# applied-ai-lab/genesis

Hardware: AMD Instinct MI355X
Metric: training images/sec (fwd+bwd+GECO step), GENESIS-V2 K=7 64x64 (higher is better)
Workload: dtype f32

## Files before the change

genesis_amd/csrc/gx_norm.hip:

```cpp
#include "gx_common.h"

#include <vector>

namespace {

struct View {
    float* ptr;
    int ctot;
    int c0;
    int mode;
    const float* proj;
    int projC;
    const float* pgate;
    int nsplit;
    size_t sstride;
};

struct InSrc {
    const float* p;
    int nsplit;
    size_t stride;
    const float* bias;
    float* ysum;
};
// ... 759 lines not shown
    double s1 = 0.0, s2 = 0.0;
    for (int tc = 0; tc < cpg; ++tc) {
        double a = 0.0, b = 0.0;
        for (int p = 0; p < P; ++p) { a += uab[2 * (tc * P + p)]; b += uab[2 * (tc * P + p) + 1]; }
        const float gmc = gamma[gidx * cpg + tc];
        s1 += b * gmc;
        s2 += a * gmc;
        if ((int)threadIdx.x == tc) {
            float* pp = part_out + ((size_t)n * C + gidx * cpg + tc) * 3;
            pp[0] = (float)a; pp[1] = (float)b;
        }
    }
    const float k1 = (float)(s1 / m), k2 = (float)(s2 / m);
    float sd = 0.f, am = 0.f;
    float gm2 = gm, bt2 = bt;
    asm volatile("" : "+v"(gm2), "+v"(bt2));
    float wacc[CT];
#pragma unroll
    for (int q = 0; q < CT; ++q) wacc[q] = 0.f;
#pragma unroll
    for (int j = 0; j < F; ++j) {
        int jo = j * 64;
        static_assert(CT == 4, "the dependency list below names four accumulators");
        if (WP) asm volatile("" : "+v"(jo) : "v"(sd), "v"(am), "v"(k1), "v"(wacc[0]), "v"(wacc[1]), "v"(wacc[2]), "v"(wacc[3]));
        else asm volatile("" : "+v"(jo) : "v"(sd), "v"(am), "v"(k1));
        f32x4 g = {0.f, 0.f, 0.f, 0.f}, o, a;
        f32x4& xv = xr[KEEP ? j : 0];
        if constexpr (!KEEP) {
            xv = src4[jo];
#pragma unroll
            for (int e = 0; e < 4; ++e) xv[e] = (xv[e] - meanf) * rstdf;
        }
#pragma unroll
        for (int e = 0; e < 4; ++e) {
            const float t = xv[e] * gm2 + bt2;
            a[e] = t > 0.f ? t : 0.f;
        }
#pragma unroll
        for (int q = 0; q < CT; ++q) {
            const f32x4 gq = gs4[q * rowq + jo];
            g += pw[q] * gq;
            if (WP) wacc[q] += (gq[0] * a[0] + gq[1] * a[1]) + (gq[2] * a[2] + gq[3] * a[3]);
        }
#pragma unroll
        for (int e = 0; e < 4; ++e) {
            const float pre = xv[e] * gm2 + bt2;
            const float gv = pre > 0.f ? g[e] : 0.f;
            const float d = rstdf * (gv * gm2 - k1 - xv[e] * k2);
            o[e] = d;
        }
        sd += (o[0] + o[1]) + (o[2] + o[3]);
        am = fmaxf(fmaxf(am, fmaxf(fabsf(o[0]), fabsf(o[1]))), fmaxf(fabsf(o[2]), fabsf(o[3])));
        dst4[jo] = o;
    }
    {
        const double v = gx_wave_sum_d((double)sd);
        if (lane == 0) usd[unit] = v;
#pragma unroll
        for (int of = 32; of >= 1; of >>= 1) am = fmaxf(am, __shfl_xor(am, of, 64));
        if (lane == 0) uam[unit] = am;
    }
    if (WP) {
#pragma unroll
        for (int q = 0; q < CT; ++q) {
            float v = wacc[q];
#pragma unroll
            for (int o = 32; o >= 1; o >>= 1) v += __shfl_xor(v, o, 64);
            if (lane == 0) uw[unit][q] = v;
        }
    }
    __syncthreads();
    if (WP) {
        for (int t = threadIdx.x; t < cpg * ctot; t += blockDim.x) {
            const int tc = t / ctot, q = t - tc * ctot;
            float v = 0.f;
            for (int p = 0; p < P; ++p) v += uw[tc * P + p][q];
            wpart[((size_t)n * ctot + q) * C + gidx * cpg + tc] = v;
        }
    }
    if ((int)threadIdx.x < cpg) {
        double s = 0.0;
        for (int p = 0; p < P; ++p) s += usd[threadIdx.x * P + p];
        part_out[((size_t)n * C + gidx * cpg + threadIdx.x) * 3 + 2] = (float)s;
    }
    if (amax_parts && threadIdx.x == 0) {
        float r = uam[0];
#pragma unroll
        for (int i = 1; i < 16; ++i) r = fmaxf(r, uam[i]);
        amax_parts[blockIdx.x] = r;
    }
}

__global__ void __launch_bounds__(1024)
gn_relu_fwd_small_kernel(const InSrc src, const float* __restrict__ gamma, const float* __restrict__ beta,
                         int C, int H, int W, int groups, float eps, View d0, View d1,
                         float* __restrict__ mean_out, float* __restrict__ rstd_out) {
    __shared__ double red[16 * 2 + 2];
    const int n = blockIdx.x / groups, gidx = blockIdx.x % groups;
    const int cpg = C / groups, HW = H * W;
    const int m = cpg * HW;
    const int e = threadIdx.x * 4;
    const bool act = e < m;
    const size_t slab_off = ((size_t)n * C + (size_t)gidx * cpg) * HW;
    f32x4 v = {0.f, 0.f, 0.f, 0.f};
    if (act) v = load_in4(src, slab_off + e, gidx * cpg + e / HW);
    double acc[2];
    acc[0] = ((double)v[0] + (double)v[1]) + ((double)v[2] + (double)v[3]);
    acc[1] = ((double)v[0] * v[0] + (double)v[1] * v[1]) + ((double)v[2] * v[2] + (double)v[3] * v[3]);
    block_sum_multi<2>(acc, red);
    const double mean = acc[0] / m;
    double var = acc[1] / m - mean * mean;
    if (var < 0.0) var = 0.0;
    const float meanf = (float)mean;
    const float rstdf = (float)(1.0 / sqrt(var + (double)eps));
    if (threadIdx.x == 0) { mean_out[blockIdx.x] = meanf; rstd_out[blockIdx.x] = rstdf; }
    if (act && d0.ptr) {
        const int cl = e / HW, hw = e - cl * HW;
        const int c = gidx * cpg + cl;
        const int r = hw / W, col = hw - r * W;
        const float gm = gamma[c], bt = beta[c];
        f32x4 o;
#pragma unroll
        for (int u = 0; u < 4; ++u) {
            const float t = (v[u] - meanf) * rstdf * gm + bt;
            o[u] = t > 0.f ? t : 0.f;
        }
        store_view4(d0, n, c, r, col, H, W, o);
        if (d1.ptr) store_view4(d1, n, c, r, col, H, W, o);
    }
}

__global__ void __launch_bounds__(1024)
gn_relu_bwd_small_kernel(const float* __restrict__ y, const float* __restrict__ gamma, const float* __restrict__ beta,
                         const float* __restrict__ mean_in, const float* __restrict__ rstd_in,
                         int C, int H, int W, int groups, View g0, View g1,
                         float* __restrict__ dy, float* __restrict__ part_out) {
    __shared__ double ta[1024], tb[1024];
    __shared__ double ca[64], cb[64];
    const int n = blockIdx.x / groups, gidx = blockIdx.x % groups;
    const int cpg = C / groups, HW = H * W;
    const int m = cpg * HW;
    const int tpc = HW >> 2;
    const int e = threadIdx.x * 4;
    const bool act = e < m;
    const size_t slab_off = ((size_t)n * C + (size_t)gidx * cpg) * HW;
    const float meanf = mean_in[blockIdx.x], rstdf = rstd_in[blockIdx.x];
    int cl = 0, c = gidx * cpg, r = 0, col = 0;
    f32x4 xh = {0.f, 0.f, 0.f, 0.f}, gv = {0.f, 0.f, 0.f, 0.f};
    float gm = 0.f;
    double a = 0.0, b = 0.0;
    if (act) {
        cl = e / HW;
        const int hw = e - cl * HW;
        c = gidx * cpg + cl;
        r = hw / W; col = hw - r * W;
        const f32x4 xv = reinterpret_cast<const f32x4*>(y + slab_off)[threadIdx.x];
        f32x4 g = load_view4(g0, n, c, r, col, H, W);
        if (g1.ptr) { const f32x4 g2 = load_view4(g1, n, c, r, col, H, W); g += g2; }
        gm = gamma[c];
        const float bt = beta[c];
#pragma unroll
        for (int u = 0; u < 4; ++u) {
            const float h = (xv[u] - meanf) * rstdf;
            const float pre = h * gm + bt;
            const float gg = pre > 0.f ? g[u] : 0.f;
            xh[u] = h; gv[u] = gg;
            a += (double)gg * h;
            b += (double)gg;
        }
    }
    ta[threadIdx.x] = a; tb[threadIdx.x] = b;
    __syncthreads();
    if ((int)threadIdx.x < cpg) {
        double sa = 0.0, sb = 0.0;
        for (int i = 0; i < tpc; ++i) { sa += ta[threadIdx.x * tpc + i]; sb += tb[threadIdx.x * tpc + i]; }
        ca[threadIdx.x] = sa; cb[threadIdx.x] = sb;
        float* pp = part_out + ((size_t)n * C + gidx * cpg + threadIdx.x) * 3;
        pp[0] = (float)sa; pp[1] = (float)sb;
    }
    __syncthreads();
    double s1 = 0.0, s2 = 0.0;
    for (int i = 0; i < cpg; ++i) {
        const float gi = gamma[gidx * cpg + i];
        s1 += cb[i] * gi;
        s2 += ca[i] * gi;
    }
    const float k1 = (float)(s1 / m), k2 = (float)(s2 / m);
    double sd = 0.0;
    if (act) {
        f32x4 o;
#pragma unroll
        for (int u = 0; u < 4; ++u) {
            const float d = rstdf * (gv[u] * gm - k1 - xh[u] * k2);
            o[u] = d;
            sd += d;
        }
        reinterpret_cast<f32x4*>(dy + slab_off)[threadIdx.x] = o;
    }
    __syncthreads();
    ta[threadIdx.x] = sd;
    __syncthreads();
    if ((int)threadIdx.x < cpg) {
        double s = 0.0;
        for (int i = 0; i < tpc; ++i) s += ta[threadIdx.x * tpc + i];
        part_out[((size_t)n * C + gidx * cpg + threadIdx.x) * 3 + 2] = (float)s;
    }
}

int small_threads(int cpg, int H, int W) {
    const int HW = H * W, m = cpg * HW;
    if (HW >= 256 || (W % 4) != 0 || cpg > 64 || m > 4096) return 0;
    return gx_round_up(m / 4, 64);
}

inline float* gn_take_link_out(const float* tensor, int ctot, int c0, int mode, int C, unsigned nwg, size_t covered, bool second_copy = false) {
    GxAmaxLink& L = gx_amax_link();
    const bool link_ok = !second_copy && L.parts && !L.tensor && tensor && c0 == 0 && mode == 0 && ctot == C && covered == L.numel;
    return gx_amax_producer_out(tensor, link_ok, nwg, covered);
}
template <int F, int UPW>
void launch_fwd_reg(dim3 grid, dim3 block, hipStream_t s, const InSrc src, const float* gamma, const float* beta, int C, int H,
                    int W, int groups, int P, float eps, View d0, View d1, float* mean, float* rstd) {
    float* ap = d0.ptr ? gn_take_link_out(d0.ptr, d0.ctot, d0.c0, d0.mode, C, grid.x, (size_t)(grid.x / groups) * C * H * W, d1.ptr != nullptr) : nullptr;
    hipLaunchKernelGGL((gn_relu_fwd_reg_kernel<F, UPW>), grid, block, 0, s, src, gamma, beta, C, H, W, groups, P, eps, d0, d1,
                       mean, rstd, ap);
}
template <int F, int UPW>
bool launch_bwd_stage(dim3 grid, dim3 block, hipStream_t s, size_t lds, const float* y, const float* gamma,
                      const float* beta, const float* mean, const float* rstd, int C, int H, int W, int groups, int P,
                      View g0, View g1, float* dy, float* part, float* wpart, float* bpart) {
    if (UPW != 1 || block.x != 1024 || g0.ctot != 4) return false;
    float* amax_parts = gn_take_link_out(dy, C, 0, 0, C, grid.x, (size_t)(grid.x / groups) * C * H * W);
    constexpr bool KEEP = F < 8;
    static bool attr_set = false;
    if (!attr_set) {
        (void)hipFuncSetAttribute(reinterpret_cast<const void*>(&gn_relu_bwd_stage_kernel<F, 4, true, KEEP>),
                                  hipFuncAttributeMaxDynamicSharedMemorySize, 150 * 1024);
        (void)hipFuncSetAttribute(reinterpret_cast<const void*>(&gn_relu_bwd_stage_kernel<F, 4, false, KEEP>),
                                  hipFuncAttributeMaxDynamicSharedMemorySize, 150 * 1024);
        attr_set = true;
    }
#define GX_STAGE_LAUNCH(WP_)                                                                                               \
    hipLaunchKernelGGL((gn_relu_bwd_stage_kernel<F, 4, WP_, KEEP>), grid, block, lds, s, y, gamma, beta, mean, rstd, C, H, W, \
                       groups, P, g0, g1, dy, part, wpart, bpart, amax_parts)
    if (wpart) GX_STAGE_LAUNCH(true); else GX_STAGE_LAUNCH(false);
#undef GX_STAGE_LAUNCH
    return true;
}

template <int F, int UPW>
void launch_bwd_reg(dim3 grid, dim3 block, hipStream_t s, size_t lds, const float* y, const float* gamma, const float* beta,
                    const float* mean, const float* rstd, int C, int H, int W, int groups, int P, View g0, View g1, float* dy,
                    float* part, float* wpart, float* bpart) {
    if (!lds) {
        float* ap = gn_take_link_out(dy, C, 0, 0, C, grid.x, (size_t)(grid.x / groups) * C * H * W);
        hipLaunchKernelGGL((gn_relu_bwd_reg_kernel<F, UPW, false>), grid, block, 0, s, y, gamma, beta, mean, rstd, C, H, W, groups,
                           P, g0, g1, dy, part, wpart, bpart, ap);
        return;
    }
    static bool attr_set = false;
    if (!attr_set) {
        (void)hipFuncSetAttribute(reinterpret_cast<const void*>(&gn_relu_bwd_reg_kernel<F, UPW, true>),
                                  hipFuncAttributeMaxDynamicSharedMemorySize, 150 * 1024);
        attr_set = true;
    }
    if (launch_bwd_stage<F, UPW>(grid, block, s, lds, y, gamma, beta, mean, rstd, C, H, W, groups, P, g0, g1, dy, part, wpart, bpart))
        return;
    float* ap = gn_take_link_out(dy, C, 0, 0, C, grid.x, (size_t)(grid.x / groups) * C * H * W);
    hipLaunchKernelGGL((gn_relu_bwd_reg_kernel<F, UPW, true>), grid, block, lds, s, y, gamma, beta, mean, rstd, C, H, W, groups, P,
                       g0, g1, dy, part, wpart, bpart, ap);
}

#define GX_GN_REG_DISPATCH(LAUNCH, pl, ...)                                      \
    do {                                                                         \
        if (pl.UPW == 1) {                                                       \
            if (pl.F == 1) LAUNCH<1, 1>(__VA_ARGS__);                            \
            else if (pl.F == 2) LAUNCH<2, 1>(__VA_ARGS__);                       \
            else if (pl.F == 4) LAUNCH<4, 1>(__VA_ARGS__);                       \
            else LAUNCH<8, 1>(__VA_ARGS__);                                      \
        } else {                                                                 \
            if (pl.F == 1) LAUNCH<1, 2>(__VA_ARGS__);                            \
            else if (pl.F == 2) LAUNCH<2, 2>(__VA_ARGS__);                       \
            else LAUNCH<4, 2>(__VA_ARGS__);                                      \
        }                                                                        \
    } while (0)

struct GnRedTable { GxGnRed e[48]; };
__global__ void __launch_bounds__(256)
gn_param_reduce_batch_kernel(const GnRedTable tab) {
    const GxGnRed& r = tab.e[blockIdx.y];
    const int c = blockIdx.x;
    if (c >= r.C) return;
    __shared__ double red[16 * 3 + 3];
    double v[3] = {0.0, 0.0, 0.0};
    for (int n = threadIdx.x; n < r.N; n += blockDim.x) {
        const float* p = r.part + ((size_t)n * r.C + c) * 3;
        v[0] += p[0]; v[1] += p[1]; v[2] += p[2];
    }
    block_sum_multi<3>(v, red);
    if (threadIdx.x == 0) {
        r.dgamma[c] += (float)v[0];
        r.dbeta[c] += (float)v[1];
        if (r.dbias) r.dbias[c] += (float)v[2];
    }
}

int check_view(const char* name, const View& v, int C) {
    GX_CHECK_ARG(v.mode >= 0 && v.mode <= 2, "%s: bad view mode %d", name, v.mode);
    GX_CHECK_ARG(v.c0 >= 0 && v.c0 + C <= v.ctot, "%s: view slice [%d,%d) outside %d channels", name, v.c0,
                 v.c0 + C, v.ctot);
    return GX_OK;
}

constexpr int kSplitPix = 4096;
constexpr int kSplitRec = 3 * 8 + 8 * 8 + 8;
// ... 282 lines not shown
         d1{dst1, dst1_ctot, dst1_c0, dst1_mode, nullptr, 0, nullptr};
    int rc = dst0 ? check_view("gx_gn_relu_fwd", d0, C) : GX_OK;
    if (rc) return rc;
    if (dst1) { rc = check_view("gx_gn_relu_fwd", d1, C); if (rc) return rc; }
    const int m = (C / groups) * H * W;
    const int threads = m >= 16384 ? 1024 : (m >= 2048 ? 512 : 256);
    const bool vec = (W % 4) == 0;
    {
        auto vw = [](int mode) { return mode == 1 ? 4.0 : (mode == 2 ? 0.25 : 1.0); };
        const double el = (double)N * C * H * W;
        GxProf pf(KID_GN_FWD, (hipStream_t)stream, 8.0 * el,
                  4.0 * el * (src.nsplit + (src.ysum ? 1.0 : 0.0) + (dst0 ? vw(dst0_mode) : 0.0) +
                              (dst1 ? vw(dst1_mode) : 0.0)));
        const RegPlan pl = plan_reg(C / groups, H, W);
        const int st = small_threads(C / groups, H, W);
        if (pl.ok)
            GX_GN_REG_DISPATCH(launch_fwd_reg, pl, dim3(N * groups), dim3(pl.threads), (hipStream_t)stream, src, gamma,
                               beta, C, H, W, groups, pl.P, eps, d0, d1, mean, rstd);
        else if (st)
            hipLaunchKernelGGL(gn_relu_fwd_small_kernel, dim3(N * groups), dim3(st), 0, (hipStream_t)stream, src, gamma,
                               beta, C, H, W, groups, eps, d0, d1, mean, rstd);
        else {
            float* ap = dst0 ? gn_take_link_out(dst0, d0.ctot, d0.c0, d0.mode, C, (unsigned)(N * groups), (size_t)N * C * H * W, dst1 != nullptr) : nullptr;
            if (vec)
                hipLaunchKernelGGL(gn_relu_fwd_kernel<true>, dim3(N * groups), dim3(threads), 0, (hipStream_t)stream, src,
                                   gamma, beta, C, H, W, groups, eps, d0, d1, mean, rstd, ap);
            else
                hipLaunchKernelGGL(gn_relu_fwd_kernel<false>, dim3(N * groups), dim3(threads), 0, (hipStream_t)stream, src,
                                   gamma, beta, C, H, W, groups, eps, d0, d1, mean, rstd, ap);
        }
    }
    GX_CHECK_LAUNCH("gx_gn_relu_fwd");
    return GX_OK;
}

size_t gx_gn_relu_bwd_ws_bytes(int N, int C) { return (size_t)N * C * 3 * sizeof(float); }
size_t gx_gn_relu_bwd_proj_ws_bytes(int N, int C, int H, int W, int groups, int Cout) {
    size_t b = gx_gn_relu_bwd_ws_bytes(N, C);
    if (proj_split_ok(C, H, W, groups, Cout))
        b += ((size_t)N * groups * (H * W / kSplitPix) * kSplitRec + (size_t)N * groups * 2) * sizeof(float);
    return b;
}

static int gn_relu_bwd_impl(const float* y, const float* gamma, const float* beta, const float* mean,
                            const float* rstd, int N, int C, int H, int W, int groups, const View& v0, const View& v1,
                            float* dy, float* dgamma, float* dbeta, float* dbias, void* ws, size_t ws_bytes,
                            gx_stream_t stream, float* wpart = nullptr, float* bpart = nullptr);

int gx_gn_relu_bwd(const float* y, const float* gamma, const float* beta, const float* mean, const float* rstd,
                   int N, int C, int H, int W, int groups, const float* g0, int g0_ctot, int g0_c0, int g0_mode,
                   const float* g1, int g1_ctot, int g1_c0, int g1_mode, float* dy, float* dgamma, float* dbeta,
                   float* dbias, void* ws, size_t ws_bytes, gx_stream_t stream) {
    return gx_gn_relu_bwd_parts(y, gamma, beta, mean, rstd, N, C, H, W, groups, g0, g0_ctot, g0_c0, g0_mode, 1, 0, g1, g1_ctot,
                                g1_c0, g1_mode, 1, 0, dy, dgamma, dbeta, dbias, ws, ws_bytes, stream);
}

int gx_gn_relu_bwd_parts(const float* y, const float* gamma, const float* beta, const float* mean, const float* rstd,
                         int N, int C, int H, int W, int groups, const float* g0, int g0_ctot, int g0_c0, int g0_mode,
                         int g0_nsplit, size_t g0_split_stride, const float* g1, int g1_ctot, int g1_c0, int g1_mode,
                         int g1_nsplit, size_t g1_split_stride, float* dy, float* dgamma, float* dbeta, float* dbias, void* ws,
                         size_t ws_bytes, gx_stream_t stream) {
    GX_CHECK_ARG(g0, "gx_gn_relu_bwd: null pointer");
    GX_CHECK_ARG(g0_nsplit >= 1 && g1_nsplit >= 1, "gx_gn_relu_bwd_parts: nsplit >= 1");
    View v0{const_cast<float*>(g0), g0_ctot, g0_c0, g0_mode, nullptr, 0, nullptr, g0_nsplit, g0_split_stride},
         v1{const_cast<float*>(g1), g1_ctot, g1_c0, g1_mode, nullptr, 0, nullptr, g1_nsplit, g1_split_stride};
    int rc = check_view("gx_gn_relu_bwd", v0, C);
    if (rc) return rc;
    if (g1) { rc = check_view("gx_gn_relu_bwd", v1, C); if (rc) return rc; }
    return gn_relu_bwd_impl(y, gamma, beta, mean, rstd, N, C, H, W, groups, v0, v1, dy, dgamma, dbeta, dbias, ws,
                            ws_bytes, stream);
}

int gx_gn_relu_bwd_proj(const float* y, const float* gamma, const float* beta, const float* mean, const float* rstd,
                        int N, int C, int H, int W, int groups, const float* g_out, int Cout, const float* w,
                        const float* gate, float* dy, float* dgamma, float* dbeta, float* dbias, float* wpart,
                        float* bpart, void* ws, size_t ws_bytes, gx_stream_t stream) {
    GX_CHECK_ARG(g_out && w, "gx_gn_relu_bwd_proj: null pointer");
    GX_CHECK_ARG((wpart == nullptr) == (bpart == nullptr), "gx_gn_relu_bwd_proj: wpart and bpart go together");
    GX_CHECK_ARG(Cout >= 1 && Cout <= 8, "gx_gn_relu_bwd_proj: Cout must be 1..8 (got %d)", Cout);
    GX_CHECK_ARG((W % 4) == 0 && ((uintptr_t)g_out % 16) == 0, "gx_gn_relu_bwd_proj: W %% 4 == 0 and 16-byte alignment");
    View v0{const_cast<float*>(g_out), Cout, 0, 3, w, C, gate}, v1{nullptr, 0, 0, 0, nullptr, 0, nullptr};
    return gn_relu_bwd_impl(y, gamma, beta, mean, rstd, N, C, H, W, groups, v0, v1, dy, dgamma, dbeta, dbias, ws,
                            ws_bytes, stream, wpart, bpart);
}

int gx_gn_relu_bwd_proj_fuses_wgrad(int C, int H, int W, int groups, int Cout) {
    if (C <= 0 || groups <= 0 || C % groups || Cout < 1 || Cout > 8 || (C / groups) * Cout > 1024) return 0;
    if (!gx_is_pow2(H) || !gx_is_pow2(W)) return 0;
    if (proj_split_ok(C, H, W, groups, Cout)) return 1;
    return plan_reg(C / groups, H, W).ok && (size_t)Cout * H * W * 4 <= 128 * 1024;
}

static int gn_relu_bwd_impl(const float* y, const float* gamma, const float* beta, const float* mean,
                            const float* rstd, int N, int C, int H, int W, int groups, const View& v0, const View& v1,
                            float* dy, float* dgamma, float* dbeta, float* dbias, void* ws, size_t ws_bytes,
                            gx_stream_t stream, float* wpart, float* bpart) {
    const float* g1 = v1.ptr;
    const int g0_mode = v0.mode, g1_mode = v1.mode;
    GX_CHECK_ARG(y && gamma && beta && mean && rstd && dy && dgamma && dbeta && ws,
                 "gx_gn_relu_bwd: null pointer");
    GX_CHECK_ARG(N > 0 && C > 0 && groups > 0 && C % groups == 0,
                 "gx_gn_relu_bwd: bad N/C/groups");
    GX_CHECK_ARG(gx_is_pow2(H) && gx_is_pow2(W) && W >= 2 && H >= 2, "gx_gn_relu_bwd: H,W must be powers of two >= 2");
    GX_CHECK_ARG(ws_bytes >= gx_gn_relu_bwd_ws_bytes(N, C), "gx_gn_relu_bwd: workspace too small");
    const int hw = H * W;
    const bool vec = (W % 4) == 0;
    const int threads = hw >= 4096 ? 1024 : (hw >= 1024 ? 256 : 64);
    hipStream_t s = (hipStream_t)stream;
    {
        auto vw = [](int mode) { return mode == 1 ? 4.0 : (mode == 2 ? 0.25 : (mode == 3 ? 0.0 : 1.0)); };
        const double el = (double)N * C * H * W;
        GxProf pf(KID_GN_BWD, s, 16.0 * el, 4.0 * el * (2.0 + vw(g0_mode) + (g1 ? vw(g1_mode) : 0.0)));
        const RegPlan pl = plan_reg(C / groups, H, W);
        const int st = small_threads(C / groups, H, W);
        if (v0.mode == 3 && !g1 && proj_split_ok(C, H, W, groups, v0.ctot) &&
            ws_bytes >= gx_gn_relu_bwd_proj_ws_bytes(N, C, H, W, groups, v0.ctot)) {
            const int chunks = hw / kSplitPix;
            float* rec = (float*)ws + (size_t)N * C * 3;
            float* kk = rec + (size_t)N * groups * chunks * kSplitRec;
            const dim3 grid(N * groups * chunks);
            if (v0.ctot <= 4)
                hipLaunchKernelGGL(gn_bwd_proj_split_sums_kernel<4>, grid, dim3(256), 0, s, y, gamma, beta, mean, rstd, C, hw,
                                   groups, v0, rec);
            else
                hipLaunchKernelGGL(gn_bwd_proj_split_sums_kernel<8>, grid, dim3(256), 0, s, y, gamma, beta, mean, rstd, C, hw,
                                   groups, v0, rec);
            hipLaunchKernelGGL(gn_bwd_proj_split_combine_kernel, dim3(N * groups), dim3(64), 0, s, (const float*)rec, gamma, rstd,
                               C, hw, groups, chunks, v0.ctot, kk, (float*)ws, wpart, bpart);
            float* ap = gn_take_link_out(dy, C, 0, 0, C, grid.x, (size_t)N * C * H * W);
            if (v0.ctot <= 4)
                hipLaunchKernelGGL(gn_bwd_proj_split_apply_kernel<4>, grid, dim3(256), 0, s, y, gamma, beta, mean, rstd, C, hw,
                                   groups, v0, (const float*)kk, dy, ap);
            else
                hipLaunchKernelGGL(gn_bwd_proj_split_apply_kernel<8>, grid, dim3(256), 0, s, y, gamma, beta, mean, rstd, C, hw,
                                   groups, v0, (const float*)kk, dy, ap);
        }
        else if (pl.ok) {
            const size_t stage = (v0.mode == 3 && (size_t)v0.ctot * hw * 4 <= 128 * 1024) ? (size_t)v0.ctot * hw * 4 : 0;
            GX_CHECK_ARG(!wpart || stage, "gx_gn_relu_bwd_proj: fused 1x1 weight gradient unsupported for this shape");
            GX_GN_REG_DISPATCH(launch_bwd_reg, pl, dim3(N * groups), dim3(pl.threads), s, stage, y, gamma, beta, mean,
                               rstd, C, H, W, groups, pl.P, v0, v1, dy, (float*)ws, wpart, bpart);
        }
        else if (wpart)
            GX_CHECK_ARG(false, "gx_gn_relu_bwd_proj: fused 1x1 weight gradient unsupported for this shape");
        else if (st)
            hipLaunchKernelGGL(gn_relu_bwd_small_kernel, dim3(N * groups), dim3(st), 0, s, y, gamma, beta, mean, rstd,
                               C, H, W, groups, v0, v1, dy, (float*)ws);
        else {
            float* ap = gx_amax_producer_out(dy, false, (unsigned)(N * groups), (size_t)N * C * H * W);
            if (vec)
                hipLaunchKernelGGL(gn_relu_bwd_kernel<true>, dim3(N * groups), dim3(threads), 0, s, y, gamma, beta, mean,
                                   rstd, C, H, W, groups, v0, v1, dy, (float*)ws, ap);
            else
                hipLaunchKernelGGL(gn_relu_bwd_kernel<false>, dim3(N * groups), dim3(threads), 0, s, y, gamma, beta, mean,
                                   rstd, C, H, W, groups, v0, v1, dy, (float*)ws, ap);
        }
    }
    GX_CHECK_LAUNCH("gx_gn_relu_bwd");
    if (g_gx_defer_on) {
        const GxGnRed rec{(const float*)ws, dgamma, dbeta, dbias, N, C};
        if (gx_defer_push_gn(rec)) return GX_OK;
        return gx_defer_flush_gn(&rec, 1, s);
    }
    {
        GxProf pf(KID_GN_PARAM_REDUCE, s, 0.0, 12.0 * N * C);
        hipLaunchKernelGGL(gn_param_reduce_kernel, dim3(C), dim3(N >= 128 ? 256 : 64), 0, s, (const float*)ws, N, C,
// ... 21 lines not shown
```

genesis_amd/hip_ops.py:

```python
import ctypes
import os

import torch

from . import _lib
from ._lib import GenesisHipError

F32 = torch.float32
KERNELS = {'gaussian': 0, 'laplacian': 1, 'epanechnikov': 2}


def _chk(t, name, dtype=F32):
    if t is None:
        return
    if not t.is_cuda:
        raise GenesisHipError('%s: the HIP hot path needs device tensors (got %s); there is no CPU fallback'
                              % (name, t.device))
    if t.dtype != dtype:
        raise GenesisHipError('%s: expected %s, got %s' % (name, dtype, t.dtype))
    if not t.is_contiguous():
        raise GenesisHipError('%s: tensor must be contiguous' % name)


def _p(t):
# ... 1279 lines not shown
    key = (device.index, torch.cuda.current_stream(device).cuda_stream, which)
    t = _LSTM_BAR.get(key)
    if t is None:
        t = _LSTM_BAR[key] = torch.zeros(_lib.query('gx_lstm_seq_ws_bytes') // 4, dtype=torch.int32, device=device)
    return t


def lstm_seq_steps(B, H):
    return lstm_seq_capacity(B, H) if LSTM_SEQ else 0


def lstm_seq_capacity(B, H):
    return _lib.query('gx_lstm_seq_max_steps', B, H)


def lstm_seq_fwd(gx3, w_hh, b_hh, act, c, h):
    T, B, H4 = gx3.shape
    for t, n in ((gx3, 'gx'), (w_hh, 'w_hh'), (b_hh, 'b_hh'), (act, 'act'), (c, 'c'), (h, 'h')):
        _chk(t, 'lstm_seq_fwd.' + n)
    _lib.call('gx_lstm_seq_fwd', _p(gx3), _p(w_hh), _p(b_hh), T, B, H4 // 4, _p(act), _p(c), _p(h),
              _p(_lstm_bar(gx3.device, 0)), _stream())


def lstm_seq_bwd(g_h, w_hh, act, c, dgates, dc2):
    T, B, H4 = act.shape
    for t, n in ((g_h, 'g_h'), (w_hh, 'w_hh'), (act, 'act'), (c, 'c'), (dgates, 'dgates'), (dc2, 'dc2')):
        _chk(t, 'lstm_seq_bwd.' + n)
    _lib.call('gx_lstm_seq_bwd', _p(g_h), _p(w_hh), _p(act), _p(c), T, B, H4 // 4, _p(dgates), _p(dc2),
              _p(_lstm_bar(act.device, 1)), _stream())


def conv1x1_gn_fwd(y_pre, mean, rstd, gamma, beta, groups, w, bias, gate=None, addend=None):
    _chk(y_pre, 'conv1x1_gn.y'); _chk(mean, 'conv1x1_gn.mean'); _chk(rstd, 'conv1x1_gn.rstd')
    _chk(gamma, 'conv1x1_gn.gamma'); _chk(beta, 'conv1x1_gn.beta'); _chk(w, 'conv1x1_gn.w'); _chk(bias, 'conv1x1_gn.bias')
    _chk(gate, 'conv1x1_gn.gate'); _chk(addend, 'conv1x1_gn.addend')
    N, Cin, H, W = y_pre.shape
    Cout = w.shape[0]
    out = torch.empty(N, Cout, H, W, dtype=F32, device=y_pre.device)
    _lib.call('gx_conv1x1_gn_fwd', _p(y_pre), _p(mean), _p(rstd), _p(gamma), _p(beta), groups, _p(w), _p(bias),
              _p(gate), _p(addend), N, Cin, Cout, H, W, _p(out), _stream())
    return out


def conv1x1_gn_wgrad(y_pre, mean, rstd, gamma, beta, groups, g_out, w=None, bias=None, gate=None, out=None):
    _chk(y_pre, 'conv1x1_gn_wgrad.y'); _chk(g_out, 'conv1x1_gn_wgrad.g')
    N, Cin, H, W = y_pre.shape
    Cout = g_out.shape[1]
    o = out or (None, None, None)
    dw = o[0] if o[0] is not None else torch.empty(Cout, Cin, dtype=F32, device=y_pre.device)
    db = o[1] if o[1] is not None else torch.empty(Cout, dtype=F32, device=y_pre.device)
    dgate = (o[2] if o[2] is not None else torch.empty((), dtype=F32, device=y_pre.device)) if gate is not None else None
    _chk(dw, 'conv1x1_gn_wgrad.dw'); _chk(db, 'conv1x1_gn_wgrad.db'); _chk(dgate, 'conv1x1_gn_wgrad.dgate')
    assert dw.numel() == Cout * Cin and db.numel() == Cout
    nb = _lib.query('gx_conv1x1_gn_wgrad_ws_bytes', N, Cin, Cout, H, W)
    ws = _ws(nb, y_pre.device)
    _lib.call('gx_conv1x1_gn_wgrad', _p(y_pre), _p(mean), _p(rstd), _p(gamma), _p(beta), groups, _p(g_out), _p(w),
              _p(bias), _p(gate), N, Cin, Cout, H, W, _p(dw), _p(db), _p(dgate), _p(ws), nb, _stream())
    return dw, db, dgate


def conv1x1_gn_bwd_fused(y, gamma, beta, mean, rstd, groups, g_out, w, bias, gate=None, want_dbias=False,
                         out_gn=None, out_conv=None):
    N, C, H, W = y.shape
    Cout = int(g_out.shape[1])
    if not _lib.query('gx_gn_relu_bwd_proj_fuses_wgrad', C, H, W, groups, Cout):
        return None
    wpart = torch.empty(N, Cout, C, dtype=F32, device=y.device)
    bpart = torch.empty(N, Cout, dtype=F32, device=y.device)
    dy, dgamma, dbeta, dbias = gn_relu_bwd_proj(y, gamma, beta, mean, rstd, groups, g_out, w, want_dbias, out_gn, gate,
                                                parts=(wpart, bpart))
    o = out_conv or (None, None, None)
    dw = o[0] if o[0] is not None else torch.empty(Cout, C, dtype=F32, device=y.device)
    db = o[1] if o[1] is not None else torch.empty(Cout, dtype=F32, device=y.device)
    dgate = (o[2] if o[2] is not None else torch.empty((), dtype=F32, device=y.device)) if gate is not None else None
    _chk(dw, 'conv1x1_gn_bwd.dw'); _chk(db, 'conv1x1_gn_bwd.db'); _chk(dgate, 'conv1x1_gn_bwd.dgate')
    assert dw.numel() == Cout * C and db.numel() == Cout
    nb = _lib.query('gx_conv1x1_gn_wgrad_finish_ws_bytes', C, Cout)
    ws = _ws(nb, y.device)
    _lib.call('gx_conv1x1_gn_wgrad_finish', _p(wpart), _p(bpart), N, C, Cout, _p(w), _p(bias), _p(gate), _p(dw), _p(db),
              _p(dgate), _p(ws), nb, _stream())
    return dy, (dgamma, dbeta, dbias), (dw, db, dgate)


def gn_relu_bwd_proj(y, gamma, beta, mean, rstd, groups, g_out, w, want_dbias=False, out=None, gate=None,
                     parts=(None, None)):
    _chk(y, 'gn_bwd_proj.y'); _chk(g_out, 'gn_bwd_proj.g'); _chk(w, 'gn_bwd_proj.w')
    N, C, H, W = y.shape
    dy = torch.empty_like(y)
    o = out or (None, None, None)
    dgamma = o[0] if o[0] is not None else torch.empty(C, dtype=F32, device=y.device)
    dbeta = o[1] if o[1] is not None else torch.empty(C, dtype=F32, device=y.device)
    dbias = (o[2] if o[2] is not None else torch.empty(C, dtype=F32, device=y.device)) if want_dbias else None
    nb = _lib.query('gx_gn_relu_bwd_proj_ws_bytes', N, C, H, W, groups, int(g_out.shape[1]))
    ws = _ws(nb, y.device)
    direct = o[0] is not None and o[1] is not None and (not want_dbias or o[2] is not None)
    tap = _tap_begin(y.device, H * W, y.numel())
    with _deferring(direct, ws):
        _lib.call('gx_gn_relu_bwd_proj', _p(y), _p(gamma), _p(beta), _p(mean), _p(rstd), N, C, H, W, groups,
                  _p(g_out), int(g_out.shape[1]), _p(w), _p(gate), _p(dy), _p(dgamma), _p(dbeta), _p(dbias),
                  _p(parts[0]), _p(parts[1]), _p(ws), nb, _stream())
    _tap_end(tap)
    return dy, dgamma, dbeta, dbias


def conv3x3_pair_supported(x, w1, w2):
    N, Cin, H, W = x.shape
    return bool(_lib.query('gx_conv3x3_pair_supported', N, Cin, w1.shape[0], w2.shape[0], H, W))


class PairWs(object):
    __slots__ = ('t', 'f16')

    def __init__(self, t, f16):
        self.t, self.f16 = t, f16


def conv3x3_pair_fwd(x, w1, w2, amax_in=None):
    _chk(x, 'pair.x'); _chk(w1, 'pair.w1'); _chk(w2, 'pair.w2')
    N, Cin, H, W = x.shape
    Co1, Co2 = w1.shape[0], w2.shape[0]
    y1 = torch.empty(N, Co1, H, W, dtype=F32, device=x.device)
    y2 = torch.empty(N, Co2, H, W, dtype=F32, device=x.device)
    nb = _lib.query('gx_conv3x3_pair_ws_bytes', N, Cin, Co1, Co2, H, W)
    ws = _ws(nb, x.device)
    hint = _input_amax(amax_in)
    with hint:
        _lib.call('gx_conv3x3_pair_fwd', _p(x), _p(w1), _p(w2), _p(y1), _p(y2), N, Cin, Co1, Co2, H, W, _p(ws), nb, _stream())
    return y1, y2, PairWs(ws, hint.on)


def conv3x3_pair_dgrad(dy1, dy2, w1, w2, ws=None, amax_in=None):
    _chk(dy1, 'pair.dy1'); _chk(dy2, 'pair.dy2'); _chk(w1, 'pair.w1'); _chk(w2, 'pair.w2')
    N, Co1, H, W = dy1.shape
    Co2, Cin = dy2.shape[1], w1.shape[1]
    dx = torch.empty(N, Cin, H, W, dtype=F32, device=dy1.device)
    nb = _lib.query('gx_conv3x3_pair_ws_bytes', N, Cin, Co1, Co2, H, W)
    hint = _input_amax(amax_in)
    if isinstance(ws, PairWs):
        ws = ws.t if ws.f16 == hint.on else None
    pack = ws is None
    if pack:
        ws = _ws(nb, dy1.device)
    with hint:
        _lib.call('gx_conv3x3_pair_dgrad', _p(dy1), _p(dy2), _p(w1), _p(w2), _p(dx), N, Cin, Co1, Co2, H, W, int(pack),
                  _p(ws), nb, _stream())
    return dx


def conv3x3_wino(x, w, mode=0, amax_in=None):
    _chk(x, 'wino.x'); _chk(w, 'wino.w')
    N, _, H, W = x.shape
    Cout, Cin = w.shape[0], w.shape[1]
    y = torch.empty(N, Cout if mode == 0 else Cin, H, W, dtype=F32, device=x.device)
    nb = _lib.query('gx_conv3x3_wino_ws_bytes', N, Cin, Cout, H, W)
    ws = _ws(nb, x.device)
    with _input_amax(amax_in):
        _lib.call('gx_conv3x3_wino', _p(x), _p(w), _p(y), N, Cin, Cout, H, W, mode, _p(ws), nb, _stream())
    return y
```

include/genesis_hip.h:

```cpp
#ifndef GENESIS_HIP_H
#define GENESIS_HIP_H
#include <stddef.h>
#include <stdint.h>

#ifdef __cplusplus
extern "C" {
#endif

typedef void* gx_stream_t;

#define GX_OK 0
#define GX_EINVAL (-1)
#define GX_ELAUNCH (-2)
#define GX_EDATA (-3)

const char* gx_last_error(void);
int gx_version(void);

size_t gx_conv3x3_ws_bytes(int N, int Cin, int Cout, int H, int W);
int gx_conv3x3_fwd(const float* x, const float* w, float* y, int N, int Cin, int Cout, int H, int W,
                   void* ws, size_t ws_bytes, gx_stream_t stream);
int gx_conv3x3_dgrad(const float* dy, const float* w, float* dx, int N, int Cin, int Cout, int H, int W,
                     void* ws, size_t ws_bytes, gx_stream_t stream);
int gx_conv3x3_dgrad_parts(const float* dy, const float* w, float* dx, int N, int Cin, int Cout, int H, int W, void* ws,
                           size_t ws_bytes, const float** parts, int* nsplit, size_t* split_stride, gx_stream_t stream);
size_t gx_conv3x3_wgrad_ws_bytes(int N, int Cin, int Cout, int H, int W);
int gx_conv3x3_wgrad(const float* x, const float* dy, float* dw, int N, int Cin, int Cout, int H, int W,
                     void* ws, size_t ws_bytes, gx_stream_t stream);

int gx_conv3x3_wino_supported(int N, int Cin, int Cout, int H, int W);
int gx_conv3x3_wino_policy(int mode);
int gx_wino_precision(int mode);
int gx_kq_policy(int mode);
int gx_wgq_policy(int mode);
int gx_wgq_precision(int mode);
int gx_wgq_operand_amax(const float* a0, int na0, const float* a1, int na1, const float* b0, int nb0, const float* b1,
                        int nb1, float* out2);
double gx_wgq_last_f16_share(void);
int gx_wgq_ring(int on);
int gx_kq_precision(int mode);
#define GX_MATMUL_MIXED 3
int gx_matmul_precision(int level);
int gx_matmul_precision_get(void);
int gx_tapconv_precision(int mode);
int gx_tapconv_precision_get(void);
int gx_tapconv_last_mode(void);
int gx_kq_amax_link(float* parts, int capacity, size_t numel);
int gx_kq_amax_link_hits(void);
int gx_amax_tap(float* parts, int capacity, size_t numel);
int gx_conv_input_amax(const float* p0, int n0, const float* p1, int n1);
double gx_wino_f16_share(void);
int gx_amax_tap_result(void);
int gx_amax_parts(const float* x, size_t n, float* parts, gx_stream_t stream);
size_t gx_conv3x3_wino_ws_bytes(int N, int Cin, int Cout, int H, int W);
int gx_conv3x3_wino(const float* x, const float* w, float* y, int N, int Cin, int Cout, int H, int W, int mode,
                    void* ws, size_t ws_bytes, gx_stream_t stream);
int gx_conv3x3_pair_supported(int N, int Cin, int Co1, int Co2, int H, int W);
size_t gx_conv3x3_pair_ws_bytes(int N, int Cin, int Co1, int Co2, int H, int W);
int gx_conv3x3_pair_fwd(const float* x, const float* w1, const float* w2, float* y1, float* y2, int N, int Cin, int Co1,
                        int Co2, int H, int W, void* ws, size_t ws_bytes, gx_stream_t stream);
int gx_conv3x3_pair_dgrad(const float* dy1, const float* dy2, const float* w1, const float* w2, float* dx, int N, int Cin,
                          int Co1, int Co2, int H, int W, int pack, void* ws, size_t ws_bytes, gx_stream_t stream);

size_t gx_deconv5x5s2_ws_bytes(int N, int Cin, int Cout, int Hin, int Win);
int gx_deconv5x5s2_fwd(const float* x, const float* w, const float* bias, float* y, int N, int Cin, int Cout,
                       int Hin, int Win, void* ws, size_t ws_bytes, gx_stream_t stream);
size_t gx_deconv5x5s2_gn_stats_ws_bytes(int N, int Cin, int Cout, int Hin, int Win);
int gx_deconv5x5s2_gn_stats_fwd(const float* x, const float* w, const float* bias, float* y, int N, int Cin, int Cout,
                                int Hin, int Win, int groups, float eps, float* mean, float* rstd, int* fused,
                                void* ws, size_t ws_bytes, gx_stream_t stream);
int gx_deconv5x5s2_dgrad(const float* dy, const float* w, float* dx, int N, int Cin, int Cin_out, int Cout,
                         int Hin, int Win, void* ws, size_t ws_bytes, gx_stream_t stream);
size_t gx_deconv5x5s2_wgrad_ws_bytes(int N, int Cin, int Cout, int Hin, int Win);
int gx_deconv5x5s2_wgrad(const float* x, const float* dy, float* dw, int N, int Cin, int Cout, int Hin, int Win,
                         void* ws, size_t ws_bytes, gx_stream_t stream);

int gx_gn_relu_fwd(const float* y, const float* gamma, const float* beta, int N, int C, int H, int W, int groups,
                   float eps, float* dst0, int dst0_ctot, int dst0_c0, int dst0_mode, float* dst1, int dst1_ctot,
                   int dst1_c0, int dst1_mode, float* mean, float* rstd, gx_stream_t stream);
size_t gx_gn_relu_bwd_ws_bytes(int N, int C);
int gx_gn_relu_bwd(const float* y, const float* gamma, const float* beta, const float* mean, const float* rstd,
                   int N, int C, int H, int W, int groups, const float* g0, int g0_ctot, int g0_c0, int g0_mode,
                   const float* g1, int g1_ctot, int g1_c0, int g1_mode, float* dy, float* dgamma, float* dbeta,
                   float* dbias, void* ws, size_t ws_bytes, gx_stream_t stream);
int gx_gn_relu_bwd_parts(const float* y, const float* gamma, const float* beta, const float* mean, const float* rstd,
                         int N, int C, int H, int W, int groups, const float* g0, int g0_ctot, int g0_c0, int g0_mode,
                         int g0_nsplit, size_t g0_split_stride, const float* g1, int g1_ctot, int g1_c0, int g1_mode,
                         int g1_nsplit, size_t g1_split_stride, float* dy, float* dgamma, float* dbeta, float* dbias, void* ws,
                         size_t ws_bytes, gx_stream_t stream);
int gx_gn_relu_bwd_proj(const float* y, const float* gamma, const float* beta, const float* mean, const float* rstd,
                        int N, int C, int H, int W, int groups, const float* g_out, int Cout, const float* w,
                        const float* gate, float* dy, float* dgamma, float* dbeta, float* dbias, float* wpart,
                        float* bpart, void* ws, size_t ws_bytes, gx_stream_t stream);
int gx_gn_relu_bwd_proj_fuses_wgrad(int C, int H, int W, int groups, int Cout);
int gx_gn_relu_active_count(const float* y, const float* gamma, const float* beta, const float* mean, const float* rstd, int N,
                            int C, int H, int W, int groups, unsigned long long* count, gx_stream_t stream);
size_t gx_gn_relu_bwd_proj_ws_bytes(int N, int C, int H, int W, int groups, int Cout);

int gx_icsbp_fwd(const float* colour, const double* log_sigma, const float* rand_pixel, const int64_t* seed_idx_in,
                 int B, int C, int H, int W, int K, int kernel_type, float* log_m, float* log_s, float* seeds,
                 int64_t* seed_idx_out, gx_stream_t stream);
size_t gx_icsbp_bwd_ws_bytes(int B, int H, int W, int K);
int gx_icsbp_bwd(const float* colour, const double* log_sigma, const float* seeds, const int64_t* seed_idx,
                 const float* g_log_m, int B, int C, int H, int W, int K, int kernel_type, float* dcolour,
                 double* dlog_sigma, void* ws, size_t ws_bytes, gx_stream_t stream);
int gx_icsbp_fwd_dyn(const float* colour, const double* log_sigma, const float* rand_pixel, const int64_t* seed_idx_in,
                     int B, int C, int H, int W, int K, int kernel_type, float min_mass, float* log_m, float* log_s,
                     float* seeds, int64_t* seed_idx_out, int* nsteps, gx_stream_t stream);
int gx_icsbp_bwd_dyn(const float* colour, const double* log_sigma, const float* seeds, const int64_t* seed_idx,
                     const float* g_log_m, const int* nsteps, int B, int C, int H, int W, int K, int kernel_type,
                     float* dcolour, double* dlog_sigma, void* ws, size_t ws_bytes, gx_stream_t stream);

int gx_maskpool_fwd(const float* f, const float* log_m, int B, int C, int H, int W, int K, float* S, float* msum,
                    gx_stream_t stream);
int gx_maskpool_bwd(const float* f, const float* log_m, const float* gS, const float* gmsum, int B, int C, int H,
                    int W, int K, float* df, float* dlog_m, gx_stream_t stream);

size_t gx_mixture_ws_bytes(int B, int H, int W);
int gx_mixture_fwd(const float* x, const float* dec, int B, int H, int W, int K, float pixel_std, int pixel_bound,
                   float* recon, float* x_r, float* log_m_r, float* err, void* ws, size_t ws_bytes,
                   gx_stream_t stream);
int gx_mixture_bwd(const float* x, const float* dec, const float* g_err, int B, int H, int W, int K,
                   float pixel_std, int pixel_bound, float* ddec, gx_stream_t stream);

int gx_conv1x1_fwd(const float* x, const float* w, const float* bias, const float* gate, const float* addend,
                   int N, int Cin, int Cout, int H, int W, float* y, gx_stream_t stream);
size_t gx_conv1x1_bwd_ws_bytes(int N, int Cin, int Cout, int H, int W);
int gx_conv1x1_bwd(const float* x, const float* dy, const float* w, const float* bias, const float* gate, int N,
                   int Cin, int Cout, int H, int W, float* dx, float* dw, float* db, float* dgate, void* ws,
                   size_t ws_bytes, gx_stream_t stream);
int gx_conv1x1_bwd_ex(const float* x, const float* dy, const float* w, const float* bias, const float* gate, int N,
                      int Cin, int Cout, int H, int W, float* dx, float* dw, float* db, float* dgate, int accumulate,
                      void* ws, size_t ws_bytes, gx_stream_t stream);
size_t gx_conv1x1_bwd_act_ws_bytes(int N, int Cin, int Cout, int H, int W);
int gx_conv1x1_bwd_act(const float* x, const float* dy, const float* w, const float* bias, int N, int Cin, int Cout, int H,
                       int W, int act, float* dxa, float* dw, float* db, float* dbx, void* ws, size_t ws_bytes,
                       gx_stream_t stream);
int gx_conv1x1_gn_fwd(const float* y_pre, const float* mean, const float* rstd, const float* gamma,
                      const float* beta, int groups, const float* w, const float* bias, const float* gate,
                      const float* addend, int N, int Cin, int Cout, int H, int W, float* out, gx_stream_t stream);
size_t gx_conv1x1_gn_wgrad_ws_bytes(int N, int Cin, int Cout, int H, int W);
int gx_conv1x1_gn_wgrad(const float* y_pre, const float* mean, const float* rstd, const float* gamma,
                        const float* beta, int groups, const float* g_out, const float* w, const float* bias,
                        const float* gate, int N, int Cin, int Cout, int H, int W, float* dw, float* db,
                        float* dgate, void* ws, size_t ws_bytes, gx_stream_t stream);
size_t gx_conv1x1_gn_wgrad_finish_ws_bytes(int Cin, int Cout);
int gx_conv1x1_gn_wgrad_finish(const float* wpart, const float* bpart, int N, int Cin, int Cout, const float* w,
                               const float* bias, const float* gate, float* dw, float* db, float* dgate, void* ws,
                               size_t ws_bytes, gx_stream_t stream);

int gx_adam_step(void* p, const void* g, void* m, void* v, size_t n, int is_f64, int64_t* step, double lr,
                 double beta1, double beta2, double eps, float grad_scale, gx_stream_t stream);
int gx_step_increment(int64_t* step, gx_stream_t stream);
int gx_philox_noise(float* u, long long nu, float* z, long long nz, unsigned long long seed, const int64_t* step,
                    gx_stream_t stream);
int gx_geco_update(float* state, const float* err, float goal, float step_size, float alpha, float speedup,
                   int use_speedup, float beta_min, float beta_max, gx_stream_t stream);
int gx_geco_update_step(float* state, const float* err, float goal, float step_size, float alpha, float speedup,
                        int use_speedup, float beta_min, float beta_max, int64_t* step, gx_stream_t stream);
int gx_adam_step_pair(float* p32, float* g32, float* m32, float* v32, size_t n32, double* p64, double* g64,
                      double* m64, double* v64, size_t n64, int64_t* step, double lr, double beta1, double beta2,
                      double eps, float grad_scale, int zero_grads, gx_stream_t stream);

int gx_optimiser_step_pair(int kind, float* p32, float* g32, float* m32, size_t n32, double* p64, double* g64, double* m64,
                           size_t n64, int64_t* step, double lr, double hp, double eps, float grad_scale, int zero_grads,
                           gx_stream_t stream);
int gx_beta_warmup(const int64_t* step, float beta, float warm_iters, float* out, gx_stream_t stream);
size_t gx_mse_rmse_ws_bytes(int B);
int gx_mse_rmse(const float* x, const float* recon, int B, int n, float* out, void* ws, size_t ws_bytes, gx_stream_t stream);

int gx_profile_enable(int on);
int gx_profile_num_kernels(void);
const char* gx_profile_kernel_name(int kid);
int gx_profile_collect(double* total_ms, double* launches, double* flops, double* bytes);

int gx_conv3x3_bias_act_fwd(const float* x, const float* w, const float* bias, int act, float* y, int N, int Cin,
                            int Cout, int H, int W, void* ws, size_t ws_bytes, gx_stream_t stream);
// ... 272 lines not shown
```

Before: 12130.

## Hold GroupNorm-ReLU backward slab in registers with 512-thread stage kernel

```diff
diff --git a/genesis_amd/csrc/gx_norm.hip b/genesis_amd/csrc/gx_norm.hip
--- a/genesis_amd/csrc/gx_norm.hip
+++ b/genesis_amd/csrc/gx_norm.hip
@@ -865,6 +865,211 @@
         double s = 0.0;
         for (int p = 0; p < P; ++p) s += usd[threadIdx.x * P + p];
         part_out[((size_t)n * C + gidx * cpg + threadIdx.x) * 3 + 2] = (float)s;
+    }
+    if (amax_parts && threadIdx.x == 0) {
+        float r = uam[0];
+#pragma unroll
+        for (int i = 1; i < 16; ++i) r = fmaxf(r, uam[i]);
+        amax_parts[blockIdx.x] = r;
+    }
+}
+
+template <int CT>
+__device__ __forceinline__ void gn_stage_pass1_f4(f32x4& xv, const f32x4* gs4, int jo, int rowq, const float (&pw)[CT],
+                                                  float meanf, float rstdf, float gm, float bt, bool fuse_sa,
+                                                  float& sa, float& sb) {
+#pragma clang fp contract(off)
+    f32x4 g = {0.f, 0.f, 0.f, 0.f};
+#pragma unroll
+    for (int e = 0; e < 4; ++e) xv[e] = (xv[e] - meanf) * rstdf;
+#pragma unroll
+    for (int q = 0; q < CT; ++q) {
+        const f32x4 gq = gs4[q * rowq + jo];
+#pragma unroll
+        for (int e = 0; e < 4; ++e) g[e] = __builtin_fmaf(pw[q], gq[e], g[e]);
+    }
+#pragma unroll
+    for (int e = 0; e < 4; ++e) {
+        const float pre = __builtin_fmaf(xv[e], gm, bt);
+        g[e] = pre > 0.f ? g[e] : 0.f;
+    }
+    if (fuse_sa) sa += __builtin_fmaf(g[0], xv[0], g[1] * xv[1]) + __builtin_fmaf(g[2], xv[2], g[3] * xv[3]);
+    else sa += (g[0] * xv[0] + g[1] * xv[1]) + (g[2] * xv[2] + g[3] * xv[3]);
+    sb += (g[0] + g[1]) + (g[2] + g[3]);
+}
+template <int CT, bool WP>
+__device__ __forceinline__ f32x4 gn_stage_pass2_f4(const f32x4& xv, const f32x4* gs4, int jo, int rowq, const float (&pw)[CT],
+                                                   float gm2, float bt2, float rstdf, float k1, float k2, bool last,
+                                                   float (&wacc)[CT], float& sd, float& am) {
+#pragma clang fp contract(off)
+    f32x4 g = {0.f, 0.f, 0.f, 0.f}, o, a, pre, t;
+#pragma unroll
+    for (int e = 0; e < 4; ++e) {
+        pre[e] = __builtin_fmaf(xv[e], gm2, bt2);
+        a[e] = pre[e] > 0.f ? pre[e] : 0.f;
+    }
+#pragma unroll
+    for (int q = 0; q < CT; ++q) {
+        const f32x4 gq = gs4[q * rowq + jo];
+#pragma unroll
+        for (int e = 0; e < 4; ++e) g[e] = __builtin_fmaf(pw[q], gq[e], g[e]);
+        if (WP) {
+            if (last) wacc[q] += __builtin_fmaf(gq[0], a[0], gq[1] * a[1]) + __builtin_fmaf(gq[2], a[2], gq[3] * a[3]);
+            else wacc[q] += __builtin_fmaf(gq[1], a[1], gq[0] * a[0]) + __builtin_fmaf(gq[2], a[2], gq[3] * a[3]);
+        }
+    }
+#pragma unroll
+    for (int e = 0; e < 4; ++e) {
+        const float gv = pre[e] > 0.f ? g[e] : 0.f;
+        t[e] = __builtin_fmaf(-xv[e], k2, __builtin_fmaf(gv, gm2, -k1));
+        o[e] = rstdf * t[e];
+    }
+    sd += __builtin_fmaf(rstdf, t[0], o[1]) + __builtin_fmaf(rstdf, t[2], o[3]);
+    am = fmaxf(fmaxf(am, fmaxf(fabsf(o[0]), fabsf(o[1]))), fmaxf(fabsf(o[2]), fabsf(o[3])));
+    return o;
+}
+
+template <int CT, bool WP>
+__global__ void __launch_bounds__(512) __attribute__((amdgpu_waves_per_eu(4, 4)))
+gn_relu_bwd_stage_regs_kernel(const float* __restrict__ y, const float* __restrict__ gamma, const float* __restrict__ beta,
+                              const float* __restrict__ mean_in, const float* __restrict__ rstd_in,
+                              int C, int groups, View g0,
+                              float* __restrict__ dy, float* __restrict__ part_out, float* __restrict__ wpart,
+                              float* __restrict__ bpart, float* __restrict__ amax_parts) {
+    constexpr int F = 8, P = 2, HW = F * 256 * P, rowq = HW >> 2, q4 = rowq / P;
+    const int slab_id = gx_xcd_tile(blockIdx.x, gridDim.x);
+    __shared__ double uab[16 * 2];
+    __shared__ double usd[16];
+    __shared__ float uam[16];
+    __shared__ float uw[16][8];
+    extern __shared__ __attribute__((aligned(16))) float gsl[];
+    const int n = slab_id / groups, gidx = slab_id % groups;
+    const int cpg = C / groups;
+    const int m = cpg * HW;
+    const int lane = threadIdx.x & 63, cl = threadIdx.x >> 6;
+    const int c = gidx * cpg + cl;
+    const size_t slab_off = ((size_t)n * C + (size_t)gidx * cpg) * HW;
+    const f32x4* src4 = reinterpret_cast<const f32x4*>(y + slab_off) + cl * rowq + lane;
+    f32x4* dst4 = reinterpret_cast<f32x4*>(dy + slab_off) + cl * rowq + lane;
+    const f32x4* gs4 = reinterpret_cast<const f32x4*>(gsl) + lane;
+    f32x4 xr[P][F];
+#pragma unroll
+    for (int p = 0; p < P; ++p)
+#pragma unroll
+        for (int j = 0; j < F; ++j) xr[p][j] = src4[p * q4 + j * 64];
+    const float meanf = mean_in[slab_id], rstdf = rstd_in[slab_id];
+    {
+        const f32x4* g4 = reinterpret_cast<const f32x4*>(g0.ptr + (size_t)n * CT * HW);
+#pragma unroll 4
+        for (int i = 0; i < (CT * rowq) / 512; ++i)
+            reinterpret_cast<f32x4*>(gsl)[i * 512 + threadIdx.x] = g4[i * 512 + threadIdx.x];
+    }
+    __syncthreads();
+    float pw[CT];
+    {
+        const float gt = g0.pgate ? *g0.pgate : 1.f;
+#pragma unroll
+        for (int q = 0; q < CT; ++q)
+            pw[q] = __builtin_bit_cast(float, __builtin_amdgcn_readfirstlane(__builtin_bit_cast(int, gt * g0.proj[q * g0.projC + c])));
+    }
+    const float gm = gamma[c], bt = beta[c];
+    float sa[P], sb[P];
+#pragma unroll
+    for (int p = 0; p < P; ++p) sa[p] = sb[p] = 0.f;
+#pragma unroll
+    for (int j = 0; j < F; ++j) {
+#pragma unroll
+        for (int p = 0; p < P; ++p) {
+            int jo = p * q4 + j * 64;
+            asm volatile("" : "+v"(jo) : "v"(sa[p]), "v"(sb[p]));
+            gn_stage_pass1_f4<CT>(xr[p][j], gs4, jo, rowq, pw, meanf, rstdf, gm, bt, j != 1 && j != 4, sa[p], sb[p]);
+        }
+    }
+#pragma unroll
+    for (int p = 0; p < P; ++p) {
+        const int unit = cl * P + p;
+        const double a = gx_wave_sum_d((double)sa[p]);
+        const double b = gx_wave_sum_d((double)sb[p]);
+        if (lane == 0) { uab[2 * unit] = a; uab[2 * unit + 1] = b; }
+    }
+    __syncthreads();
+    double s1 = 0.0, s2 = 0.0;
+    for (int tc = 0; tc < cpg; ++tc) {
+        double a = 0.0, b = 0.0;
+        for (int p = 0; p < P; ++p) { a += uab[2 * (tc * P + p)]; b += uab[2 * (tc * P + p) + 1]; }
+        const float gmc = gamma[gidx * cpg + tc];
+        s1 += b * gmc;
+        s2 += a * gmc;
+        if ((int)threadIdx.x == tc) {
+            float* pp = part_out + ((size_t)n * C + gidx * cpg + tc) * 3;
+            pp[0] = (float)a; pp[1] = (float)b;
+        }
+    }
+    const float k1 = (float)(s1 / m), k2 = (float)(s2 / m);
+    float sd[P], am[P], wacc[P][CT];
+#pragma unroll
+    for (int p = 0; p < P; ++p) {
+        sd[p] = am[p] = 0.f;
+#pragma unroll
+        for (int q = 0; q < CT; ++q) wacc[p][q] = 0.f;
+    }
+    float gm2 = gm, bt2 = bt;
+    asm volatile("" : "+v"(gm2), "+v"(bt2));
+#pragma unroll
+    for (int j = 0; j < F; ++j) {
+#pragma unroll
+        for (int p = 0; p < P; ++p) {
+            int jo = p * q4 + j * 64;
+            static_assert(CT == 4, "the dependency list below names four accumulators");
+            if (WP) asm volatile("" : "+v"(jo) : "v"(sd[p]), "v"(am[p]), "v"(k1), "v"(wacc[p][0]), "v"(wacc[p][1]), "v"(wacc[p][2]), "v"(wacc[p][3]));
+            else asm volatile("" : "+v"(jo) : "v"(sd[p]), "v"(am[p]), "v"(k1));
+            dst4[jo] = gn_stage_pass2_f4<CT, WP>(xr[p][j], gs4, jo, rowq, pw, gm2, bt2, rstdf, k1, k2, j == F - 1, wacc[p], sd[p], am[p]);
+        }
+    }
+#pragma unroll
+    for (int p = 0; p < P; ++p) {
+        const int unit = cl * P + p;
+        const double v = gx_wave_sum_d((double)sd[p]);
+        if (lane == 0) usd[unit] = v;
+        float a = am[p];
+#pragma unroll
+        for (int of = 32; of >= 1; of >>= 1) a = fmaxf(a, __shfl_xor(a, of, 64));
+        if (lane == 0) uam[unit] = a;
+        if (WP) {
+#pragma unroll
+            for (int q = 0; q < CT; ++q) {
+                float w = wacc[p][q];
+#pragma unroll
+                for (int o = 32; o >= 1; o >>= 1) w += __shfl_xor(w, o, 64);
+                if (lane == 0) uw[unit][q] = w;
+            }
+        }
+    }
+    __syncthreads();
+    if (WP) {
+        for (int t = threadIdx.x; t < cpg * CT; t += blockDim.x) {
+            const int tc = t / CT, q = t - tc * CT;
+            float v = 0.f;
+            for (int p = 0; p < P; ++p) v += uw[tc * P + p][q];
+            wpart[((size_t)n * CT + q) * C + gidx * cpg + tc] = v;
+        }
+    }
+    if ((int)threadIdx.x < cpg) {
+        double s = 0.0;
+        for (int p = 0; p < P; ++p) s += usd[threadIdx.x * P + p];
+        part_out[((size_t)n * C + gidx * cpg + threadIdx.x) * 3 + 2] = (float)s;
+    }
+    if (bpart && gidx == 0) {
+        for (int q = cl; q < CT; q += (int)(blockDim.x >> 6)) {
+            float v = 0.f;
+            for (int i = lane; i < rowq; i += 64) {
+                const f32x4 t = reinterpret_cast<const f32x4*>(gsl)[q * rowq + i];
+                v += (t[0] + t[1]) + (t[2] + t[3]);
+            }
+#pragma unroll
+            for (int o = 32; o >= 1; o >>= 1) v += __shfl_xor(v, o, 64);
+            if (lane == 0) bpart[(size_t)n * CT + q] = v;
+        }
     }
     if (amax_parts && threadIdx.x == 0) {
         float r = uam[0];
@@ -1008,12 +1213,32 @@
     hipLaunchKernelGGL((gn_relu_fwd_reg_kernel<F, UPW>), grid, block, 0, s, src, gamma, beta, C, H, W, groups, P, eps, d0, d1,
                        mean, rstd, ap);
 }
+int g_gn_stage_form = -1;
 template <int F, int UPW>
 bool launch_bwd_stage(dim3 grid, dim3 block, hipStream_t s, size_t lds, const float* y, const float* gamma,
                       const float* beta, const float* mean, const float* rstd, int C, int H, int W, int groups, int P,
                       View g0, View g1, float* dy, float* part, float* wpart, float* bpart) {
     if (UPW != 1 || block.x != 1024 || g0.ctot != 4) return false;
     float* amax_parts = gn_take_link_out(dy, C, 0, 0, C, grid.x, (size_t)(grid.x / groups) * C * H * W);
+    if constexpr (F == 8 && UPW == 1) {
+        if (P == 2 && g_gn_stage_form != 0) {
+            static bool regs_attr_set = false;
+            if (!regs_attr_set) {
+                (void)hipFuncSetAttribute(reinterpret_cast<const void*>(&gn_relu_bwd_stage_regs_kernel<4, true>),
+                                          hipFuncAttributeMaxDynamicSharedMemorySize, 150 * 1024);
+                (void)hipFuncSetAttribute(reinterpret_cast<const void*>(&gn_relu_bwd_stage_regs_kernel<4, false>),
+                                          hipFuncAttributeMaxDynamicSharedMemorySize, 150 * 1024);
+                regs_attr_set = true;
+            }
+            if (wpart)
+                hipLaunchKernelGGL((gn_relu_bwd_stage_regs_kernel<4, true>), grid, dim3(512), lds, s, y, gamma, beta, mean, rstd, C,
+                                   groups, g0, dy, part, wpart, bpart, amax_parts);
+            else
+                hipLaunchKernelGGL((gn_relu_bwd_stage_regs_kernel<4, false>), grid, dim3(512), lds, s, y, gamma, beta, mean, rstd, C,
+                                   groups, g0, dy, part, wpart, bpart, amax_parts);
+            return true;
+        }
+    }
     constexpr bool KEEP = F < 8;
     static bool attr_set = false;
     if (!attr_set) {
@@ -1462,6 +1687,13 @@
     View v0{const_cast<float*>(g_out), Cout, 0, 3, w, C, gate}, v1{nullptr, 0, 0, 0, nullptr, 0, nullptr};
     return gn_relu_bwd_impl(y, gamma, beta, mean, rstd, N, C, H, W, groups, v0, v1, dy, dgamma, dbeta, dbias, ws,
                             ws_bytes, stream, wpart, bpart);
+}
+
+int gx_gn_stage_form(int form) {
+    GX_CHECK_ARG(form == -1 || form == 0, "gx_gn_stage_form: form must be -1 (default: y held in registers where the plan allows) "
+                                          "or 0 (the two-pass form)");
+    g_gn_stage_form = form;
+    return GX_OK;
 }
 
 int gx_gn_relu_bwd_proj_fuses_wgrad(int C, int H, int W, int groups, int Cout) {
diff --git a/genesis_amd/hip_ops.py b/genesis_amd/hip_ops.py
--- a/genesis_amd/hip_ops.py
+++ b/genesis_amd/hip_ops.py
@@ -1385,6 +1385,10 @@
     return dy, (dgamma, dbeta, dbias), (dw, db, dgate)
 
 
+def gn_stage_form(form):
+    _lib.call('gx_gn_stage_form', int(form))
+
+
 def gn_relu_bwd_proj(y, gamma, beta, mean, rstd, groups, g_out, w, want_dbias=False, out=None, gate=None,
                      parts=(None, None)):
     _chk(y, 'gn_bwd_proj.y'); _chk(g_out, 'gn_bwd_proj.g'); _chk(w, 'gn_bwd_proj.w')
diff --git a/include/genesis_hip.h b/include/genesis_hip.h
--- a/include/genesis_hip.h
+++ b/include/genesis_hip.h
@@ -93,6 +93,7 @@
                         const float* gate, float* dy, float* dgamma, float* dbeta, float* dbias, float* wpart,
                         float* bpart, void* ws, size_t ws_bytes, gx_stream_t stream);
 int gx_gn_relu_bwd_proj_fuses_wgrad(int C, int H, int W, int groups, int Cout);
+int gx_gn_stage_form(int form);
 int gx_gn_relu_active_count(const float* y, const float* gamma, const float* beta, const float* mean, const float* rstd, int N,
                             int C, int H, int W, int groups, unsigned long long* count, gx_stream_t stream);
 size_t gx_gn_relu_bwd_proj_ws_bytes(int N, int C, int H, int W, int groups, int Cout);
```

After: 12250 (median of 6 runs). About the same (+1.0%).
